# davidedomini/experiments-2025-acsos-marl-for-swarming-behaviors

Measured on AMD Instinct MI355X. Metric: env-steps/sec (agents×envs), GoTo 8 agents×1024 envs @1/2/4/8 GPU, higher is better.
Workload: dtype f32; 1 GPU; GoTo train tick: 8 agents x 1024 envs/GPU, GAT, complete graph, eps 0.05, TD batch 1024 graphs/GPU; envs_per_gpu=1024, agents=8, global_envs=1024, td_batch_per_gpu=1024, graph=complete, conv=gat, parallelism=env-sharded dp1, hipgraph=True, tick=1 launch + reduce

## Files before the change

### experiments-2025-acsos-marl-for-swarming-behaviors_amd/csrc/swarm_actk.h

```cpp
#pragma once
#include "swarm_adam.h"
#include "swarm_env.h"
#include "swarm_dl.h"
#include "swarm_gat3.h"

namespace swarm {

enum { MODE_Q = 0, MODE_TICK = 1, MODE_ROLLOUT = 2, MODE_STEP = 3 };

struct ActArgs {
  int B, N, scenario, graph, k, conv, env_offset, flags;
  uint32_t k0, k1;
  float radius;
  int net;
  const float* params;
  const float* x;
  const uint8_t* dense;
  const int32_t* actions;
  float* state;
  swarm_replay replay;
  const swarm_ctrl* ctrl;
  swarm_act_out out;
  int n_ticks;
  uint32_t tick0;
// ... 246 lines not shown
      if (pending && tid == 0 && A.grad_norm_out) *A.grad_norm_out = gn;
    }
  } else if (MODE != MODE_STEP && NET == SWARM_NET_GAT3) {
    for (int i = threadIdx.x; i < G3_N_PARAMS; i += 64 * kActWPB) Pw[i] = A.params[i];
  } else if (MODE != MODE_STEP) {
    ParamStage<64 * kActWPB> ps;
    ps.load(A.params, threadIdx.x);
    ps.store(Pw, threadIdx.x);
  }
  __syncthreads();
  const float* P = Pw;
  SWARM_STAMP(1);

  const int n_ticks = (MODE == MODE_ROLLOUT) ? A.n_ticks : 1;
  float rew_sum[CT], hits_sum = 0.0f;
#pragma unroll
  for (int ct = 0; ct < CT; ++ct) rew_sum[ct] = 0.0f;

  for (int it = 0; it < n_ticks; ++it) {
#if SWARM_STAMPS == 1
    const long long t_tick0 = clock64();
#endif
    if (MODE != MODE_Q && kHoist && it > 0) pair_forces();
    if (MODE != MODE_Q) {
#pragma unroll
      for (int ct = 0; ct < CT; ++ct) {
        node_x(px[ct], py[ct], vx[ct], vy[ct], 16 * ct + c, p, F.x[ct]);
        if (!valid[ct]) { F.x[ct][0] = 0.0f; F.x[ct][1] = 0.0f; }
      }
    }
    if (MODE != MODE_STEP && NET == SWARM_NET_GAT3) {
      gat3_forward<NS>(P, d, N, graph, A.k, A.radius, A.dense, V, F);
    } else if (MODE != MODE_STEP) {
      if constexpr (kDefer) dl_forward<NS, 8, NS>(P, d, N, graph, A.k, A.radius, conv, A.dense, V, false, F, deferred0);
      else dl_forward<NS, 8>(P, d, N, graph, A.k, A.radius, conv, A.dense, V, false, F);
    }
    if constexpr (kDefer) {
      if constexpr (kDeferForces) pair_contacts0();
      if (explore0) {
#pragma unroll
        for (int ct = 0; ct < CT; ++ct) {
          const int agent = min(16 * ct + c, N - 1);
          const u32x4 wd = philox4x32(tick, genv, STREAM_RAND_ACTION, (uint32_t)(agent >> 2), A.k0, A.k1);
          const int j = agent & 3;
          ract0[ct] = uniform_int(j == 0 ? wd.x : (j == 1 ? wd.y : (j == 2 ? wd.z : wd.w)), kActions);
        }
      }
    }
    if (it == 0) SWARM_STAMP(2);

    if (MODE == MODE_Q) {
#pragma unroll
      for (int ct = 0; ct < CT; ++ct)
        if (valid[ct])
          for (int a = p; a < kActions; a += 4) A.out.q[node[ct] * kActions + a] = sm.Q[16 * ct + c][a];
      return;
    }

    const uint32_t tk = tick + (uint32_t)it;
    bool explore = explore0;
    if (it > 0 && eps > 0.0f) explore = u01(philox4x32(tk, genv, STREAM_COIN, 0u, A.k0, A.k1).x) < eps;
    int action[CT];
#pragma unroll
    for (int ct = 0; ct < CT; ++ct) {
      const int agent = min(16 * ct + c, N - 1);
      action[ct] = (MODE == MODE_STEP) ? (valid[ct] ? A.actions[node[ct]] : 0) : argmax9(F.q[ct]);
      if (explore) {
        if (kHoist && it == 0) {
// ... 192 lines not shown
```

### experiments-2025-acsos-marl-for-swarming-behaviors_amd/csrc/swarm_bwd.h

```cpp
#pragma once
#include "swarm_dl.h"

namespace swarm {

constexpr int kTdRows = 32;

template <int NS>
struct TdLds {
  static constexpr int GPB = kTdRows / NS;
  float H[kTdRows][kRow];
  float T[kTdRows][kRow];
  float R[kTdRows][kRow];
  float dZ[kTdRows][kRow];
  float dO[kTdRows][kRow];
  float dH[kTdRows][kRow];
  float X[kTdRows][9];
  union {
    struct {
      float cm[kTdRows][NS + 1];
      float dp[kTdRows][NS + 1];
    };
    WSmall<NS> tgsm[GPB];
  };
  float yq[kTdRows], gq[kTdRows], das[kTdRows], dad[kTdRows], d2[kTdRows];
// ... 30 lines not shown
  for (int t2 = 0; t2 < 2; ++t2)
#pragma unroll
    for (int r = 0; r < 4; ++r) dO[t2][r] = live ? acc[t2][r] * (1.0f - th[t2][r] * th[t2][r]) : 0.0f;
}

template <int NS>
__device__ __forceinline__ void bwd_attention(const float (*H)[kRow], const DFwd<NS>& F, const float* ssrc,
                                              const float (&dO)[DGeom<NS>::CT][2][4], const bool (&live)[DGeom<NS>::CT],
                                              int c, int p, float (&dp)[DGeom<NS>::CT][DGeom<NS>::CT][4],
                                              float (&da_d)[DGeom<NS>::CT]) {
  constexpr int CT = DGeom<NS>::CT;
  static_assert(NS % 16 == 0, "every MFMA column of a wave is one of its node slots");
  float ah[CT][2][4];
#pragma unroll
  for (int ut = 0; ut < CT; ++ut)
#pragma unroll
    for (int t = 0; t < 2; ++t) {
      const float4 hv = *reinterpret_cast<const float4*>(&H[16 * ut + c][16 * t + 4 * p]);
      ah[ut][t][0] = hv.x; ah[ut][t][1] = hv.y; ah[ut][t][2] = hv.z; ah[ut][t][3] = hv.w;
    }
#pragma unroll
  for (int ct = 0; ct < CT; ++ct) {
    float gv[CT][4], cu[CT][4];
    float part = 0.0f;
#pragma unroll
    for (int ut = 0; ut < CT; ++ut) {
      f32x4 acc = {0.f, 0.f, 0.f, 0.f};
#pragma unroll
      for (int t = 0; t < 2; ++t)
#pragma unroll
        for (int r = 0; r < 4; ++r) acc = mfma16(ah[ut][t][r], dO[ct][t][r], acc);
#pragma unroll
      for (int r = 0; r < 4; ++r) {
        float cc[4];
#pragma unroll
        for (int q = 0; q < 4; ++q) cc[q] = F.cf[ct][16 * ut + 4 * q + r];
        cu[ut][r] = pick4(cc, 0, p);
        gv[ut][r] = acc[r];
        part = part + cu[ut][r] * gv[ut][r];
      }
    }
    const float Gs = row4_sum(part);
    float dsum = 0.0f;
#pragma unroll
    for (int ut = 0; ut < CT; ++ut)
#pragma unroll
      for (int r = 0; r < 4; ++r) {
        float dpu = 0.0f;
        if (cu[ut][r] != 0.0f && live[ct]) {
          const float de = cu[ut][r] * (gv[ut][r] - Gs);
          const float pre = ssrc[16 * ut + 4 * p + r] + F.sdst[ct];
          dpu = pre > 0.0f ? de : de * kLeakySlope;
        }
        dsum = dsum + dpu;
        dp[ct][ut][r] = dpu;
      }
    da_d[ct] = row4_sum(dsum);
  }
}

template <int NS, int GS>
__device__ __forceinline__ void bwd_dh(TdLds<NS>& TB, const float* P, int row0, int N, int conv,
                                       const bool (&nv)[DGeom<NS>::CT], const float (&da_d)[DGeom<NS>::CT], int c, int p) {
  constexpr int CT = DGeom<NS>::CT;
  const float4 s0 = *reinterpret_cast<const float4*>(P + L_ATT_SRC + 4 * p);
  const float4 s1 = *reinterpret_cast<const float4*>(P + L_ATT_SRC + 16 + 4 * p);
  const float4 d0 = *reinterpret_cast<const float4*>(P + L_ATT_DST + 4 * p);
  const float4 d1 = *reinterpret_cast<const float4*>(P + L_ATT_DST + 16 + 4 * p);
  const float as[2][4] = {{s0.x, s0.y, s0.z, s0.w}, {s1.x, s1.y, s1.z, s1.w}};
  const float ad[2][4] = {{d0.x, d0.y, d0.z, d0.w}, {d1.x, d1.y, d1.z, d1.w}};
  float ao[2][NS / 4];
#pragma unroll
  for (int t = 0; t < 2; ++t)
#pragma unroll
    for (int ks = 0; ks < NS / 4; ++ks) ao[t][ks] = TB.dO[row0 + 4 * ks + p][16 * t + c];
#pragma unroll
  for (int ct = 0; ct < CT; ++ct) {
    const int u = 16 * ct + c;
    float da_s = 0.0f;
    if (conv == SWARM_CONV_GAT) {
      const int base = (GS < NS) ? (u / GS) * GS : 0;
      float dpj[GS];
#pragma unroll
      for (int j = 0; j < GS; ++j) dpj[j] = TB.dp[row0 + base + j][u];
#pragma unroll
      for (int j = 0; j < GS; ++j) asm volatile("" : "+v"(dpj[j]));
// ... 61 lines not shown
```

### experiments-2025-acsos-marl-for-swarming-behaviors_amd/csrc/swarm_common.h

```cpp
#pragma once
#include <hip/hip_runtime.h>
#include <stdint.h>

#include "../../include/swarm_hip.h"

namespace swarm {

constexpr int kHidden = 32;
constexpr int kFeat = 7;
constexpr int kActions = 9;

constexpr float kGoalX = -0.8f, kGoalY = 0.8f;
constexpr float kObstX = -0.1f, kObstY = 0.1f;
constexpr float kRadius = 0.05f;
constexpr float kCollisionForce = 100.0f;
constexpr float kContactMargin = 0.001f;
constexpr float kMinDist = 1e-6f;
constexpr float kDt = 0.1f;
constexpr float kDragKeep = 0.75f;
constexpr float kLeakySlope = 0.2f;
constexpr float kFlockShaping = 10.0f;
constexpr float kFlockDesired = 0.15f;
constexpr float kFlockContact = 0.005f;
constexpr float kFlockGoalBonus = 50.0f;
// ... 195 lines not shown
    __builtin_amdgcn_sched_barrier(0);                                                        \
    if (g_swarm_stamps && (threadIdx.x & 63) == 0)                                            \
      g_swarm_stamps[((size_t)blockIdx.x * 16 + (threadIdx.x >> 6)) * 32 + (k)] = _t;         \
  } while (0)
#define SWARM_RTSTAMP(k) SWARM_STAMP_AT(k, "s_memrealtime")
#endif
#if SWARM_STAMPS == 1
#define SWARM_STAMP(k) SWARM_STAMP_AT(k, "s_memtime")
#else
#define SWARM_STAMP(k) \
  do {              \
  } while (0)
#endif
#if !SWARM_STAMPS
#define SWARM_RTSTAMP(k) \
  do {                \
  } while (0)
#endif

enum { SPEC_RUNTIME = 0, SPEC_COMPLETE_GAT = 1, SPEC_COMPLETE_GCN = 2, SPEC_KNN_GAT = 3, SPEC_RADIUS_GAT = 4 };
__host__ __device__ inline int spec_of(int graph, int conv) {
  if (graph == SWARM_GRAPH_COMPLETE) return conv == SWARM_CONV_GAT ? SPEC_COMPLETE_GAT : SPEC_COMPLETE_GCN;
  if (graph == SWARM_GRAPH_KNN && conv == SWARM_CONV_GAT) return SPEC_KNN_GAT;
  if (graph == SWARM_GRAPH_RADIUS && conv == SWARM_CONV_GAT) return SPEC_RADIUS_GAT;
  return SPEC_RUNTIME;
}
template <int SPEC>
__device__ inline int spec_graph(int runtime) {
  return SPEC == SPEC_RUNTIME       ? runtime
         : SPEC == SPEC_KNN_GAT     ? (int)SWARM_GRAPH_KNN
         : SPEC == SPEC_RADIUS_GAT  ? (int)SWARM_GRAPH_RADIUS
                                    : (int)SWARM_GRAPH_COMPLETE;
}
template <int SPEC>
__device__ inline int spec_conv(int runtime) {
  return SPEC == SPEC_RUNTIME ? runtime : (SPEC == SPEC_COMPLETE_GCN ? (int)SWARM_CONV_GCN : (int)SWARM_CONV_GAT);
}

}
```

### experiments-2025-acsos-marl-for-swarming-behaviors_amd/csrc/swarm_dl.h

```cpp
#pragma once
#include "swarm_wpg.h"

namespace swarm {

__device__ inline float row4_sum(float x) {
  const int xi = __float_as_int(x);
  const auto a = __builtin_amdgcn_permlane16_swap(xi, xi, false, false);
  const float y = __int_as_float((int)a[0]) + __int_as_float((int)a[1]);
  const int yi = __float_as_int(y);
  const auto b = __builtin_amdgcn_permlane32_swap(yi, yi, false, false);
  return __int_as_float((int)b[0]) + __int_as_float((int)b[1]);
}

template <int M>
__device__ inline float pick4(const float (&v)[M], int k, int p) {
  const float a = v[4 * k], b = v[4 * k + 1], c = v[4 * k + 2], d = v[4 * k + 3];
  return p == 0 ? a : (p == 1 ? b : (p == 2 ? c : d));
}

template <int NS>
struct DGeom {
  static constexpr int CT = (NS + 15) / 16;
  int lane, c, p;
  int gid;
  bool live;
};

template <int NS>
__device__ inline DGeom<NS> make_dgeom(int wave_gid, int count) {
  DGeom<NS> d;
  d.lane = threadIdx.x & 63;
  d.c = d.lane & 15;
  d.p = d.lane >> 4;
  d.live = wave_gid < count;
  d.gid = d.live ? wave_gid : 0;
  return d;
}

template <int NS>
struct DFwd {
  static constexpr int CT = DGeom<NS>::CT;
  float x[CT][2];
  float t[CT][2][4];
  float zr[CT][2][4];
  float cf[CT][NS];
  float sdst[CT];
  float q[CT][kActions];
};

__device__ inline void node_x(float px, float py, float vx, float vy, int agent, int p, float x[2]) {
  x[0] = p == 0 ? px : (p == 1 ? py : (p == 2 ? vx : vy));
  x[1] = p == 0 ? kGoalX : (p == 1 ? kGoalY : (p == 2 ? (float)agent : 0.0f));
}

template <int NS, int GS = NS>
__device__ inline int in_mult(int u, int n, int N, int graph, const WSmall<NS>& sm, const uint8_t* __restrict__ dense,
                              int gid) {
  if constexpr (GS < NS) {
    if (u / GS != n / GS) return 0;
  }
  const int ju = (GS < NS) ? u % GS : u, jn = (GS < NS) ? n % GS : n;
  if (ju >= N || jn >= N) return 0;
  if (graph == SWARM_GRAPH_COMPLETE) return (ju != jn ? 1 : 0) + ((ju == 0 && jn == 0) ? 1 : 0);
  if (graph == SWARM_GRAPH_KNN)
    return (int)((sm.knn[u] >> jn) & 1u) + (int)((sm.knn[n] >> ju) & 1u) + ((ju == 0 && jn == 0) ? 1 : 0);
  if (graph == SWARM_GRAPH_RADIUS)
    return (int)((sm.knn[n] >> ju) & 1u) + ((ju == 0 && jn == 0) ? 1 : 0);
  return (int)dense[((size_t)gid * N + ju) * N + jn];
}

template <int NS, int GS = NS>
__device__ inline void in_mults(int n, int N, int graph, const WSmall<NS>& sm, const uint8_t* __restrict__ dense,
                                int gid, int m[GS]) {
  const int jn = (GS < NS) ? n % GS : n;
  const int base = (GS < NS) ? (n / GS) * GS : 0;
  const bool tv = jn < N;
  if (graph == SWARM_GRAPH_COMPLETE) {
#pragma unroll
    for (int j = 0; j < GS; ++j) m[j] = (tv && j < N) ? (int)(j != jn) + (int)(j == 0 && jn == 0) : 0;
  } else if (graph == SWARM_GRAPH_KNN) {
    const uint32_t kn = sm.knn[min(n, NS - 1)];
#pragma unroll
    for (int j = 0; j < GS; ++j)
      m[j] = (tv && j < N) ? (int)((sm.knn[base + j] >> jn) & 1u) + (int)((kn >> j) & 1u) + (int)(j == 0 && jn == 0) : 0;
  } else if (graph == SWARM_GRAPH_RADIUS) {
    const uint32_t kn = sm.knn[min(n, NS - 1)];
#pragma unroll
    for (int j = 0; j < GS; ++j) m[j] = (tv && j < N) ? (int)((kn >> j) & 1u) + (int)(j == 0 && jn == 0) : 0;
  } else {
#pragma unroll
    for (int j = 0; j < GS; ++j) m[j] = (tv && j < N) ? (int)dense[((size_t)gid * N + j) * N + jn] : 0;
  }
}

template <int NS, int GS = NS>
__device__ inline uint32_t radius_mask_node(int n, int N, float r, const WSmall<NS>& sm) {
  const int base = (GS < NS) ? (n / GS) * GS : 0;
  const int jn = (GS < NS) ? n % GS : n;
  if (jn >= N) return 0u;
  const float xi = sm.px[n], yi = sm.py[n];
  uint32_t m = 0u;
#pragma unroll
  for (int j = 0; j < GS; ++j) {
    const float d = norm2(sm.px[base + j] - xi, sm.py[base + j] - yi);
    m |= (j < N && j != jn && d <= r) ? (1u << j) : 0u;
  }
  return m;
}

template <int NS, int GS = NS>
__device__ inline uint32_t knn_mask_node(int n, int N, int k, const WSmall<NS>& sm, KV* q) {
  float d[GS];
// ... 173 lines not shown
  const unsigned long long tb = __ballot(run);
  if (tb != 0ull) {
#if SWARM_STAMPS == 1
    const long long s0 = clock64();
#endif
    wave_lds_sync();
    knn_tie_rows_wave<NS, GS>(lane, N, k, tb, LPN, sm, dn, q);
    wave_lds_sync();
    if (memo && run) {
      memo->sig_lo[n] = sig_lo;
      memo->sig_hi[n] = sig_hi;
      memo->mask[n] = sm.knn[n];
    }
#if SWARM_STAMPS == 1
    wave_lds_sync();
    const long long s1 = clock64();
    if (g_swarm_stamps && lane == 0) {
      unsigned long long* ws = g_swarm_stamps + ((size_t)blockIdx.x * 16 + (threadIdx.x >> 6)) * 32;
      ws[27] += 1ull;
      ws[28] += (unsigned long long)(s1 - s0);
      if ((unsigned long long)(s1 - s0) > ws[26]) ws[26] = (unsigned long long)(s1 - s0);
    }
#endif
  }
#if SWARM_STAMPS == 1
  if (memo && g_swarm_stamps && lane == 0 && __ballot(hit) != 0ull)
    g_swarm_stamps[((size_t)blockIdx.x * 16 + (threadIdx.x >> 6)) * 32 + 18] += 1ull;
#endif
}

struct DlNoHook {
  __device__ __forceinline__ void operator()() const {}
};
template <int NS, int SB = -1, int GS = NS, class HOOK = DlNoHook>
__device__ inline void dl_forward(const float* __restrict__ P, const DGeom<NS>& d, int N, int graph, int k, float radius, int conv,
                                  const uint8_t* __restrict__ dense, const WView<NS>& V, bool keep_tr, DFwd<NS>& F,
                                  const HOOK& hook = HOOK()) {
#define DF_STAMP(i) do { if (SB >= 0) SWARM_STAMP(SB + (i)); } while (0)
  constexpr int CT = DGeom<NS>::CT;
  WSmall<NS>& sm = *V.sm;
  const int c = d.c, p = d.p;
  float h[CT][2][4];
  {
    float a0[2][2];
#pragma unroll
    for (int t = 0; t < 2; ++t) {
      a0[t][0] = P[L_W + (16 * t + c) * kFeat + p];
      a0[t][1] = P[L_W + (16 * t + c) * kFeat + 4 + p];
      asm volatile("" : "+v"(a0[t][1]));
      a0[t][1] = (4 + p < kFeat) ? a0[t][1] : 0.0f;
    }
#pragma unroll
    for (int ct = 0; ct < CT; ++ct)
#pragma unroll
      for (int t = 0; t < 2; ++t) {
        f32x4 acc = {0.f, 0.f, 0.f, 0.f};
        acc = mfma16(a0[t][0], F.x[ct][0], acc);
        acc = mfma16(a0[t][1], F.x[ct][1], acc);
#pragma unroll
        for (int r = 0; r < 4; ++r) h[ct][t][r] = acc[r];
      }
  }
  float ssrc[CT];
  {
    const float4 s0 = *reinterpret_cast<const float4*>(P + L_ATT_SRC + 4 * p);
    const float4 s1 = *reinterpret_cast<const float4*>(P + L_ATT_SRC + 16 + 4 * p);
    const float4 d0 = *reinterpret_cast<const float4*>(P + L_ATT_DST + 4 * p);
// ... 13 lines not shown
  }
#pragma unroll
  for (int ct = 0; ct < CT; ++ct) {
    const int n = 16 * ct + c;
    if (n < NS) {
      *reinterpret_cast<float4*>(&V.H[n][4 * p]) = make_float4(h[ct][0][0], h[ct][0][1], h[ct][0][2], h[ct][0][3]);
      *reinterpret_cast<float4*>(&V.H[n][16 + 4 * p]) = make_float4(h[ct][1][0], h[ct][1][1], h[ct][1][2], h[ct][1][3]);
      if (p == 0) { sm.ssrc[n] = ssrc[ct]; sm.sdst[n] = F.sdst[ct]; sm.px[n] = F.x[ct][0]; }
      if (p == 1) sm.py[n] = F.x[ct][0];
    }
  }
  wave_lds_sync();
  DF_STAMP(0);
  if (graph == SWARM_GRAPH_KNN) {
    if constexpr (NS <= 16) {
      knn_masks_wave<NS, GS>(d.lane, N, k, sm, &V.T[0][0], reinterpret_cast<KV*>(&V.R[0][0]), V.memo);
    } else {
#pragma unroll
      for (int ct = 0; ct < CT; ++ct) {
        const int n = 16 * ct + c;
        KV* q = reinterpret_cast<KV*>(&V.T[0][0]) + (n < NS ? n : 0) * GS;
        if (n < NS && p == 0) sm.knn[n] = (((GS < NS) ? n % GS : n) < N) ? knn_mask_node<NS, GS>(n, N, k, sm, q) : 0u;
      }
    }
    wave_lds_sync();
  } else if (graph == SWARM_GRAPH_RADIUS) {
#pragma unroll
    for (int ct = 0; ct < CT; ++ct) {
      const int n = 16 * ct + c;
      if (n < NS && p == 0) sm.knn[n] = radius_mask_node<NS, GS>(n, N, radius, sm);
    }
    wave_lds_sync();
  }
  if (conv == SWARM_CONV_GAT) {
#pragma unroll
    for (int ct = 0; ct < CT; ++ct) {
      const int n = 16 * ct + c, base = (GS < NS) ? (n / GS) * GS : 0;
      float e[GS];
      int m[GS];
      in_mults<NS, GS>(n, N, graph, sm, dense, d.gid, m);
      float mx[GS];
#pragma unroll
      for (int j = 0; j < GS; ++j) {
        e[j] = leaky(sm.ssrc[base + j] + F.sdst[ct]);
        mx[j] = m[j] > 0 ? e[j] : -INFINITY;
      }
#pragma unroll
      for (int w = GS / 2; w >= 1; w >>= 1)
#pragma unroll
        for (int j = 0; j < w; ++j) mx[j] = fmaxf(mx[j], mx[j + w]);
      const float emax = mx[0];
      float den = 0.0f;
#pragma unroll
      for (int j = 0; j < GS; ++j) {
        e[j] = m[j] > 0 ? __expf(e[j] - emax) : 0.0f;
        den = den + (float)m[j] * e[j];
      }
      den = den + 1e-16f;
      const float inv = 1.0f / den;
      float cl[GS];
#pragma unroll
      for (int j = 0; j < GS; ++j) cl[j] = (float)m[j] * (e[j] * inv);
#pragma unroll
      for (int u = 0; u < NS; ++u) F.cf[ct][u] = (GS == NS || u / GS == n / GS) ? cl[u % GS] : 0.0f;
    }
  } else {
    float dis[CT];
#pragma unroll
    for (int ct = 0; ct < CT; ++ct) {
      const int n = 16 * ct + c, base = (GS < NS) ? (n / GS) * GS : 0;
      float deg = 0.0f;
#pragma unroll
      for (int j = 0; j < GS; ++j)
        if (j < N) deg = deg + (base + j == n ? 1.0f : (float)in_mult<NS, GS>(base + j, n, N, graph, sm, dense, d.gid));
      const int jn = (GS < NS) ? n % GS : n;
      dis[ct] = (jn < N && deg > 0.0f) ? 1.0f / sqrtf(deg) : 0.0f;
      if (n < NS && p == 0) sm.aux[n] = dis[ct];
    }
    wave_lds_sync();
#pragma unroll
    for (int ct = 0; ct < CT; ++ct) {
      const int n = 16 * ct + c;
#pragma unroll
      for (int u = 0; u < NS; ++u) {
        const bool same = (GS == NS) || (u / GS == n / GS);
        const float w = (u == n) ? 1.0f : (float)in_mult<NS, GS>(u, n, N, graph, sm, dense, d.gid);
        const int ju = (GS < NS) ? u % GS : u, jn = (GS < NS) ? n % GS : n;
        F.cf[ct][u] = (same && ju < N && jn < N) ? (sm.aux[u] * w) * dis[ct] : 0.0f;
      }
    }
  }
  DF_STAMP(1);
  {
    float ah[2][NS / 4];
#pragma unroll
    for (int t = 0; t < 2; ++t)
#pragma unroll
      for (int ks = 0; ks < NS / 4; ++ks) ah[t][ks] = V.H[4 * ks + p][16 * t + c];
    const float4 b0 = *reinterpret_cast<const float4*>(P + L_BIAS + 4 * p);
    const float4 b1 = *reinterpret_cast<const float4*>(P + L_BIAS + 16 + 4 * p);
    const float bias[2][4] = {{b0.x, b0.y, b0.z, b0.w}, {b1.x, b1.y, b1.z, b1.w}};
#pragma unroll
    for (int ct = 0; ct < CT; ++ct) {
      f32x4 o0 = {0.f, 0.f, 0.f, 0.f}, o1 = {0.f, 0.f, 0.f, 0.f};
#pragma unroll
      for (int ks = 0; ks < NS / 4; ++ks) {
        const float b = pick4(F.cf[ct], ks, p);
        o0 = mfma16(ah[0][ks], b, o0);
        o1 = mfma16(ah[1][ks], b, o1);
      }
#pragma unroll
      for (int r = 0; r < 4; ++r) {
        F.t[ct][0][r] = tanh_fast(o0[r] + bias[0][r]);
        F.t[ct][1][r] = tanh_fast(o1[r] + bias[1][r]);
      }
      const int n = 16 * ct + c;
      if (keep_tr && n < NS) {
        *reinterpret_cast<float4*>(&V.T[n][4 * p]) = make_float4(F.t[ct][0][0], F.t[ct][0][1], F.t[ct][0][2], F.t[ct][0][3]);
        *reinterpret_cast<float4*>(&V.T[n][16 + 4 * p]) = make_float4(F.t[ct][1][0], F.t[ct][1][1], F.t[ct][1][2], F.t[ct][1][3]);
      }
    }
  }
  DF_STAMP(2);
  {
    float a1[2][2][4];
#pragma unroll
    for (int t2 = 0; t2 < 2; ++t2)
#pragma unroll
      for (int t = 0; t < 2; ++t) {
        const float4 w = *reinterpret_cast<const float4*>(P + L_W1 + (16 * t2 + c) * kWRow + 16 * t + 4 * p);
        a1[t2][t][0] = w.x; a1[t2][t][1] = w.y; a1[t2][t][2] = w.z; a1[t2][t][3] = w.w;
      }
    const float4 bb0 = *reinterpret_cast<const float4*>(P + L_B1 + 4 * p);
    const float4 bb1 = *reinterpret_cast<const float4*>(P + L_B1 + 16 + 4 * p);
    const float b1v[2][4] = {{bb0.x, bb0.y, bb0.z, bb0.w}, {bb1.x, bb1.y, bb1.z, bb1.w}};
    hook();
#pragma unroll
    for (int ct = 0; ct < CT; ++ct) {
      f32x4 z[2] = {{0.f, 0.f, 0.f, 0.f}, {0.f, 0.f, 0.f, 0.f}};
#pragma unroll
      for (int t = 0; t < 2; ++t)
#pragma unroll
        for (int r = 0; r < 4; ++r)
#pragma unroll
          for (int t2 = 0; t2 < 2; ++t2) z[t2] = mfma16(a1[t2][t][r], F.t[ct][t][r], z[t2]);
#pragma unroll
      for (int t2 = 0; t2 < 2; ++t2) {
// ... 55 lines not shown
```

### experiments-2025-acsos-marl-for-swarming-behaviors_amd/csrc/swarm_qbk.h

```cpp
#pragma once
#include "swarm_bwd.h"

namespace swarm {

struct QbArgs {
  int B, N, graph, k, conv;
  float radius;
  const float* params;
  const float* x;
  const uint8_t* mult;
  const float* dq;
  float* slabs;
  int n_slabs;
};

constexpr int kQbDqRow = 12;

template <int NS>
struct QbSmem {
  TdLds<NS> TB;
  __attribute__((aligned(16))) float Pon[N_LDS_PARAMS];
  __attribute__((aligned(16))) float DQ[kTdRows][kQbDqRow];
};

// ... 14 lines not shown
  const int conv = spec_conv<SPEC>(A.conv);
  const int row0 = wi * NS;
  const WView<NS> V{TB.H + row0, TB.T + row0, TB.R + row0, &TB.on[wi]};
  static_assert(kSlabCols == 16, "slab column blocks of 16");
  float* const slab_base = A.slabs + (size_t)vb * kSlabCols;
  const uint32_t slab_stride = (uint32_t)A.n_slabs * kSlabCols;
  auto sst = [&](int q, float v) { slab_base[(uint32_t)(q >> 4) * slab_stride + (uint32_t)(q & 15)] = v; };

  ParamStage<NT> pon;
  pon.load(A.params, threadIdx.x);
  bool nv[CT];
  DFwd<NS> F;
  float dqv[CT][kActions];
#pragma unroll
  for (int ct = 0; ct < CT; ++ct) {
    const int n = 16 * ct + c;
    const int gi = (GS < NS) ? n / GS : 0;
    const int jl = (GS < NS) ? n % GS : n;
    const int sid = vb * (kTdRows / GS) + wi * GPW + gi;
    nv[ct] = sid < B && jl < N;
    const size_t node = (size_t)min(sid, B - 1) * N + min(jl, N - 1);
    const float x0 = A.x[node * kFeat + p], x1 = A.x[node * kFeat + min(4 + p, kFeat - 1)];
    F.x[ct][0] = nv[ct] ? x0 : 0.0f;
    F.x[ct][1] = (nv[ct] && 4 + p < kFeat) ? x1 : 0.0f;
#pragma unroll
    for (int a = 0; a < kActions; ++a) {
      const float g = A.dq[node * kActions + a];
      dqv[ct][a] = nv[ct] ? g : 0.0f;
    }
  }
  pon.store(L.Pon, threadIdx.x);
  __syncthreads();

  dl_forward<NS, -1, GS>(P, d, N, graph, A.k, A.radius, conv, A.mult, V, true, F);

  float dz[CT][2][4];
#pragma unroll
  for (int ct = 0; ct < CT; ++ct) {
    float dr[2][4] = {{0.f, 0.f, 0.f, 0.f}, {0.f, 0.f, 0.f, 0.f}};
#pragma unroll
    for (int a = 0; a < kActions; ++a)
#pragma unroll
      for (int t = 0; t < 2; ++t) {
        const float4 w = *reinterpret_cast<const float4*>(P + L_W2 + a * kWRow + 16 * t + 4 * p);
        dr[t][0] = dr[t][0] + w.x * dqv[ct][a];
        dr[t][1] = dr[t][1] + w.y * dqv[ct][a];
        dr[t][2] = dr[t][2] + w.z * dqv[ct][a];
        dr[t][3] = dr[t][3] + w.w * dqv[ct][a];
      }
#pragma unroll
    for (int t = 0; t < 2; ++t)
#pragma unroll
      for (int r = 0; r < 4; ++r) dz[ct][t][r] = (nv[ct] && F.zr[ct][t][r] > 0.0f) ? dr[t][r] : 0.0f;
    const int row = row0 + 16 * ct + c;
    row_store(TB.dZ[row], p, dz[ct]);
    TB.X[row][p] = F.x[ct][0];
    TB.X[row][4 + p] = F.x[ct][1];
#pragma unroll
    for (int j = 0; j < NS / 4; ++j) TB.cm[row][4 * j + p] = pick4(F.cf[ct], j, p);
    if (p == 0) {
      TB.X[row][8] = 0.0f;
      *reinterpret_cast<float4*>(&L.DQ[row][0]) = make_float4(dqv[ct][0], dqv[ct][1], dqv[ct][2], dqv[ct][3]);
    } else if (p == 1) {
      *reinterpret_cast<float4*>(&L.DQ[row][4]) = make_float4(dqv[ct][4], dqv[ct][5], dqv[ct][6], dqv[ct][7]);
    } else if (p == 2) {
      *reinterpret_cast<float4*>(&L.DQ[row][8]) = make_float4(dqv[ct][8], 0.0f, 0.0f, 0.0f);
    }
  }

  float dO[CT][2][4];
#pragma unroll
  for (int ct = 0; ct < CT; ++ct) {
    bwd_dO_tile(P, c, p, dz[ct], F.t[ct], nv[ct], dO[ct]);
    row_store(TB.dO[row0 + 16 * ct + c], p, dO[ct]);
  }
  float da_d[CT];
#pragma unroll
  for (int ct = 0; ct < CT; ++ct) da_d[ct] = 0.0f;
  if (conv == SWARM_CONV_GAT) {
    float dp[CT][CT][4];
    bwd_attention<NS>(TB.H + row0, F, V.sm->ssrc, dO, nv, c, p, dp, da_d);
#pragma unroll
    for (int ct = 0; ct < CT; ++ct)
#pragma unroll
      for (int ut = 0; ut < CT; ++ut)
#pragma unroll
        for (int r = 0; r < 4; ++r) TB.dp[row0 + 16 * ct + c][16 * ut + 4 * p + r] = dp[ct][ut][r];
  }
  wave_lds_sync();
  bwd_dh<NS, GS>(TB, P, row0, N, conv, nv, da_d, c, p);
  __syncthreads();

// ... 59 lines not shown
```

### experiments-2025-acsos-marl-for-swarming-behaviors_amd/csrc/swarm_tdk.h

```cpp
#pragma once
#include "swarm_adam.h"
#include "swarm_bwd.h"
#include "swarm_diag.h"

namespace swarm {

struct TdArgs {
  int S, B, N, graph, k, conv, env_offset;
  uint32_t k0, k1;
  float radius;
  const float* params;
  const float* target;
  swarm_replay replay;
  const swarm_ctrl* ctrl;
  const int32_t* sample_in;
  int32_t* sample_out;
  float* slabs;
  float gamma;
  float grad_scale;
  int n_slabs;
};

__device__ inline void slab_st(float* p, float v) { *p = v; }

// ... 232 lines not shown
        okc[ct] = true;
        if (ho[ct]) {
          okc[ct] = !kHoForceDrop && !(kHoDropTarget && !online) && (uint32_t)(g[ct][0] >> 32) == tag &&
                    (uint32_t)(g[ct][1] >> 32) == tag && (uint32_t)(g[ct][2] >> 32) == tag &&
                    (uint32_t)(g[ct][3] >> 32) == tag;
          ok = ok && okc[ct];
          st[ct] = make_float4(__uint_as_float((uint32_t)g[ct][0]), __uint_as_float((uint32_t)g[ct][1]),
                               __uint_as_float((uint32_t)g[ct][2]), __uint_as_float((uint32_t)g[ct][3]));
        }
      }
      if (!__builtin_amdgcn_ballot_w64(!ok)) break;
      if (kHoForceDrop || (kHoDropTarget && !online) || spin >= kHoSpinLimit) {
        drop_overrun<NS, GS>(okc, live_drop, nv, c);
        if (FUSED && !online && p == 0) {
#pragma unroll
          for (int ct = 0; ct < CT; ++ct)
            if (live_drop[ct]) *(volatile int*)&TB.tdrop[row0 + 16 * ct + c] = 1;
        }
        if (lane == 0) atomicAdd(X.ho_err, 1u);
        break;
      }
      __builtin_amdgcn_s_sleep(SWARM_HO_SLEEP);
    }
    SWARM_RTSTAMP(10);
    __builtin_amdgcn_s_setprio(3);
  }
  DFwd<NS> F;
#pragma unroll
  for (int ct = 0; ct < CT; ++ct) {
    node_x(st[ct].x, st[ct].y, st[ct].z, st[ct].w, jl[ct], p, F.x[ct]);
    if (!nv[ct]) { F.x[ct][0] = 0.0f; F.x[ct][1] = 0.0f; }
  }
  if (!online && !waited) __builtin_amdgcn_s_setprio(2);
  dl_forward<NS, 16, GS>(online ? Pon : Ptg, d, N, graph, A.k, A.radius, conv, nullptr, V, online, F);
  if (FUSED && waited && online) {
    for (int spin = 0;; ++spin) {
      bool ok = true, okc[CT];
#pragma unroll
      for (int ct = 0; ct < CT; ++ct) {
        okc[ct] = true;
        if (ho[ct] && !live_drop[ct]) {
          const unsigned long long g = ld_granule(ho_at(ct, 9 * N, 1));
          okc[ct] = !kHoForceDrop && (uint32_t)(g >> 32) == tag;
          ok = ok && okc[ct];
          act[ct] = nv[ct] ? (int)(uint32_t)g : 0;
        }
      }
      if (!__builtin_amdgcn_ballot_w64(!ok)) break;
      if (kHoForceDrop || spin >= kHoSpinLimit) {
        if (lane == 0) atomicAdd(X.ho_err, 1u);
        drop_overrun<NS, GS>(okc, live_drop, nv, c);
        break;
      }
      __builtin_amdgcn_s_sleep(1);
    }
    if (p == 0) {
#pragma unroll
      for (int ct = 0; ct < CT; ++ct) TB.act[row0 + 16 * ct + c] = nv[ct] ? act[ct] : 0;
    }
  }
  float dO1[CT][2][4], dp1[CT][CT][4], dad1[CT];
  if (pre) {
#pragma unroll
    for (int ct = 0; ct < CT; ++ct) {
      const int ac = min(max(act[ct], 0), kActions - 1);
      float dz1[2][4];
#pragma unroll
// ... 58 lines not shown
      if (FUSED) TB.tdrop[row0 + 16 * ct + c] = live_drop[ct] ? 1 : 0;
    }
  }
  if (!online && !waited) __builtin_amdgcn_s_setprio(0);
  if (online && lane == 0) TB.prew[wi] = pre ? 1 : 0;
  SWARM_STAMP(3);
  __syncthreads();
  SWARM_STAMP(4);

  const float* P = Pon;
  float dz[CT][2][4];
  if (online) {
#pragma unroll
    for (int ct = 0; ct < CT; ++ct) {
      const int row = row0 + 16 * ct + c;
      if (FUSED && TB.tdrop[row]) nv[ct] = false;
      float qa = F.q[ct][0];
#pragma unroll
      for (int a = 1; a < kActions; ++a) qa = (act[ct] == a) ? F.q[ct][a] : qa;
      const float delta = nv[ct] ? (qa - (rew[ct] + TB.yq[row])) : 0.0f;
      const float gq = delta * A.grad_scale;
#pragma unroll
      for (int t = 0; t < 2; ++t) {
        const float4 w = *reinterpret_cast<const float4*>(P + L_W2 + act[ct] * kWRow + 16 * t + 4 * p);
        float wv[4] = {w.x, w.y, w.z, w.w};
        asm volatile("" : "+v"(wv[0]), "+v"(wv[1]), "+v"(wv[2]), "+v"(wv[3]));
#pragma unroll
        for (int r = 0; r < 4; ++r) dz[ct][t][r] = F.zr[ct][t][r] > 0.0f ? wv[r] * gq : 0.0f;
      }
      row_store(TB.dZ[row], p, dz[ct]);
      TB.X[row][p] = F.x[ct][0];
      TB.X[row][4 + p] = F.x[ct][1];
#pragma unroll
      for (int j = 0; j < NS / 4; ++j) TB.cm[row][4 * j + p] = pick4(F.cf[ct], j, p);
      if (p == 0) { TB.X[row][8] = 0.0f; TB.gq[row] = gq; TB.d2[row] = delta * delta; }
      if (pre) {
        float o[2][4];
#pragma unroll
        for (int t = 0; t < 2; ++t)
#pragma unroll
          for (int r = 0; r < 4; ++r) o[t][r] = nv[ct] ? dO1[ct][t][r] * gq : 0.0f;
        row_store(TB.dO[row], p, o);
        if (conv == SWARM_CONV_GAT) {
#pragma unroll
          for (int ut = 0; ut < CT; ++ut)
#pragma unroll
            for (int r = 0; r < 4; ++r) TB.dp[row][16 * ut + 4 * p + r] = nv[ct] ? dp1[ct][ut][r] * gq : 0.0f;
        }
        dad1[ct] = nv[ct] ? dad1[ct] * gq : 0.0f;
      }
    }
  }
  __syncthreads();
  SWARM_STAMP(5);
  int np_pre = 0;
#pragma unroll
  for (int w2 = 0; w2 < GPB; ++w2) np_pre += TB.prew[w2];
  auto b2_tiles = [&](int tj) {
    float a1[2][8], b1[8], a2[8], b2v[8];
    int an[8];
#pragma unroll
    for (int s = 0; s < 8; ++s) {
      const int n = 4 * s + p;
      a1[0][s] = TB.dZ[n][c];
      a1[1][s] = TB.dZ[n][16 + c];
      b1[s] = TB.T[n][16 * tj + c];
      b2v[s] = TB.R[n][16 * tj + c];
// ... 101 lines not shown
```

Baseline: 625.7 million agent-steps/s.

## Compute only lane-picked GAT coefficients and specialise complete-graph softmax

Replaces the full per-node coefficient table (cf[CT][NS]) with only the entries each lane actually consumes: column picks for the aggregation MFMA and row picks for the backward attention. The picks are selected with a two-level select, and compile-time proofs check that they match the original table. A UNIT template path for complete-graph specs drops the integer multiplicity arrays and multiplies, deriving edges from a constexpr predicate. The aggregation MFMAs are also split from the tanh epilogue. The aim is to cut register pressure and per-lane ALU work in the forward pass used by the act, TD and Q-backward kernels, at the cost of more template complexity.

Result: faster. 638.1 million agent-steps/s, median of 6 (+2.0%).

```diff
diff --git a/experiments-2025-acsos-marl-for-swarming-behaviors_amd/csrc/swarm_actk.h b/experiments-2025-acsos-marl-for-swarming-behaviors_amd/csrc/swarm_actk.h
--- a/experiments-2025-acsos-marl-for-swarming-behaviors_amd/csrc/swarm_actk.h
+++ b/experiments-2025-acsos-marl-for-swarming-behaviors_amd/csrc/swarm_actk.h
@@ -302,8 +302,8 @@
     if (MODE != MODE_STEP && NET == SWARM_NET_GAT3) {
       gat3_forward<NS>(P, d, N, graph, A.k, A.radius, A.dense, V, F);
     } else if (MODE != MODE_STEP) {
-      if constexpr (kDefer) dl_forward<NS, 8, NS>(P, d, N, graph, A.k, A.radius, conv, A.dense, V, false, F, deferred0);
-      else dl_forward<NS, 8>(P, d, N, graph, A.k, A.radius, conv, A.dense, V, false, F);
+      if constexpr (kDefer) dl_forward<NS, 8, NS, spec_complete_graph(SPEC)>(P, d, N, graph, A.k, A.radius, conv, A.dense, V, false, F, deferred0);
+      else dl_forward<NS, 8, NS, spec_complete_graph(SPEC)>(P, d, N, graph, A.k, A.radius, conv, A.dense, V, false, F);
     }
     if constexpr (kDefer) {
       if constexpr (kDeferForces) pair_contacts0();
diff --git a/experiments-2025-acsos-marl-for-swarming-behaviors_amd/csrc/swarm_bwd.h b/experiments-2025-acsos-marl-for-swarming-behaviors_amd/csrc/swarm_bwd.h
--- a/experiments-2025-acsos-marl-for-swarming-behaviors_amd/csrc/swarm_bwd.h
+++ b/experiments-2025-acsos-marl-for-swarming-behaviors_amd/csrc/swarm_bwd.h
@@ -86,10 +86,7 @@
         for (int r = 0; r < 4; ++r) acc = mfma16(ah[ut][t][r], dO[ct][t][r], acc);
 #pragma unroll
       for (int r = 0; r < 4; ++r) {
-        float cc[4];
-#pragma unroll
-        for (int q = 0; q < 4; ++q) cc[q] = F.cf[ct][16 * ut + 4 * q + r];
-        cu[ut][r] = pick4(cc, 0, p);
+        cu[ut][r] = F.cr[ct][ut][r];
         gv[ut][r] = acc[r];
         part = part + cu[ut][r] * gv[ut][r];
       }
@@ -100,12 +97,10 @@
     for (int ut = 0; ut < CT; ++ut)
 #pragma unroll
       for (int r = 0; r < 4; ++r) {
-        float dpu = 0.0f;
-        if (cu[ut][r] != 0.0f && live[ct]) {
-          const float de = cu[ut][r] * (gv[ut][r] - Gs);
-          const float pre = ssrc[16 * ut + 4 * p + r] + F.sdst[ct];
-          dpu = pre > 0.0f ? de : de * kLeakySlope;
-        }
+        const float de = cu[ut][r] * (gv[ut][r] - Gs);
+        const float pre = ssrc[16 * ut + 4 * p + r] + F.sdst[ct];
+        const float dpe = pre > 0.0f ? de : de * kLeakySlope;
+        const float dpu = (cu[ut][r] != 0.0f && live[ct]) ? dpe : 0.0f;
         dsum = dsum + dpu;
         dp[ct][ut][r] = dpu;
       }
diff --git a/experiments-2025-acsos-marl-for-swarming-behaviors_amd/csrc/swarm_common.h b/experiments-2025-acsos-marl-for-swarming-behaviors_amd/csrc/swarm_common.h
--- a/experiments-2025-acsos-marl-for-swarming-behaviors_amd/csrc/swarm_common.h
+++ b/experiments-2025-acsos-marl-for-swarming-behaviors_amd/csrc/swarm_common.h
@@ -251,6 +251,7 @@
          : SPEC == SPEC_RADIUS_GAT  ? (int)SWARM_GRAPH_RADIUS
                                     : (int)SWARM_GRAPH_COMPLETE;
 }
+constexpr bool spec_complete_graph(int spec) { return spec == SPEC_COMPLETE_GAT || spec == SPEC_COMPLETE_GCN; }
 template <int SPEC>
 __device__ inline int spec_conv(int runtime) {
   return SPEC == SPEC_RUNTIME ? runtime : (SPEC == SPEC_COMPLETE_GCN ? (int)SWARM_CONV_GCN : (int)SWARM_CONV_GAT);
diff --git a/experiments-2025-acsos-marl-for-swarming-behaviors_amd/csrc/swarm_dl.h b/experiments-2025-acsos-marl-for-swarming-behaviors_amd/csrc/swarm_dl.h
--- a/experiments-2025-acsos-marl-for-swarming-behaviors_amd/csrc/swarm_dl.h
+++ b/experiments-2025-acsos-marl-for-swarming-behaviors_amd/csrc/swarm_dl.h
@@ -1,4 +1,6 @@
 #pragma once
+#include <type_traits>
+
 #include "swarm_wpg.h"
 
 namespace swarm {
@@ -12,11 +14,54 @@
   return __int_as_float((int)b[0]) + __int_as_float((int)b[1]);
 }
 
-template <int M>
-__device__ inline float pick4(const float (&v)[M], int k, int p) {
-  const float a = v[4 * k], b = v[4 * k + 1], c = v[4 * k + 2], d = v[4 * k + 3];
-  return p == 0 ? a : (p == 1 ? b : (p == 2 ? c : d));
-}
+template <class T>
+__device__ __forceinline__ T sel4(bool b0, bool b1, T x0, T x1, T x2, T x3) {
+  const T lo = b0 ? x1 : x0, hi = b0 ? x3 : x2;
+  return b1 ? hi : lo;
+}
+
+template <int NS, int GS>
+struct CoefPick {
+  static constexpr int CT = (NS + 15) / 16;
+  static_assert(GS % 4 == 0 && NS % GS == 0, "a pick's four candidates lie in one graph, 1 or 4 apart");
+  static constexpr int col_j(int ks, int q) { return (4 * ks) % GS + q; }
+  static constexpr int col_g(int ks) { return (4 * ks) / GS; }
+  static constexpr int row_j(int ut, int q, int r) { return (16 * ut + 4 * q) % GS + r; }
+  static constexpr int row_g(int ut, int q) { return (16 * ut + 4 * q) / GS; }
+  static constexpr bool same(int u, int n) { return u / GS == n / GS; }
+  static constexpr bool proved() {
+    for (int ct = 0; ct < CT; ++ct)
+      for (int c = 0; c < 16; ++c)
+        for (int p = 0; p < 4; ++p) {
+          const int n = 16 * ct + c;
+          for (int ks = 0; ks < NS / 4; ++ks) {
+            const int u = 4 * ks + p, j = col_j(ks, p);
+            if (j < 0 || j >= GS) return false;
+            if ((col_g(ks) == n / GS) != same(u, n)) return false;
+            if (same(u, n) && j != u % GS) return false;
+          }
+          if (NS % 16 != 0) continue;
+          for (int ut = 0; ut < CT; ++ut)
+            for (int r = 0; r < 4; ++r) {
+              const int u = 16 * ut + 4 * p + r, j = row_j(ut, p, r);
+              if (u >= NS || j < 0 || j >= GS) return false;
+              if ((row_g(ut, p) == n / GS) != same(u, n)) return false;
+              if (same(u, n) && j != u % GS) return false;
+            }
+        }
+    return true;
+  }
+};
+
+constexpr int complete_mult(int j, int jn) { return (int)(j != jn) + (int)(j == 0 && jn == 0); }
+constexpr bool complete_edge(int j, int jn) { return j == 0 || j != jn; }
+constexpr bool complete_mult_is_edge(int gs) {
+  for (int j = 0; j < gs; ++j)
+    for (int jn = 0; jn < gs; ++jn)
+      if (complete_mult(j, jn) != (complete_edge(j, jn) ? 1 : 0)) return false;
+  return true;
+}
+static_assert(complete_mult_is_edge(32), "complete graph: multiplicity == in-edge predicate, 0 or 1");
 
 template <int NS>
 struct DGeom {
@@ -43,7 +88,8 @@
   float x[CT][2];
   float t[CT][2][4];
   float zr[CT][2][4];
-  float cf[CT][NS];
+  float cc[CT][NS / 4];
+  float cr[CT][CT][4];
   float sdst[CT];
   float q[CT][kActions];
 };
@@ -77,7 +123,7 @@
   const bool tv = jn < N;
   if (graph == SWARM_GRAPH_COMPLETE) {
 #pragma unroll
-    for (int j = 0; j < GS; ++j) m[j] = (tv && j < N) ? (int)(j != jn) + (int)(j == 0 && jn == 0) : 0;
+    for (int j = 0; j < GS; ++j) m[j] = (tv && j < N) ? complete_mult(j, jn) : 0;
   } else if (graph == SWARM_GRAPH_KNN) {
     const uint32_t kn = sm.knn[min(n, NS - 1)];
 #pragma unroll
@@ -317,7 +363,7 @@
 struct DlNoHook {
   __device__ __forceinline__ void operator()() const {}
 };
-template <int NS, int SB = -1, int GS = NS, class HOOK = DlNoHook>
+template <int NS, int SB = -1, int GS = NS, bool UNIT = false, class HOOK = DlNoHook>
 __device__ inline void dl_forward(const float* __restrict__ P, const DGeom<NS>& d, int N, int graph, int k, float radius, int conv,
                                   const uint8_t* __restrict__ dense, const WView<NS>& V, bool keep_tr, DFwd<NS>& F,
                                   const HOOK& hook = HOOK()) {
@@ -397,47 +443,82 @@
     }
     wave_lds_sync();
   }
+  using CP = CoefPick<NS, GS>;
+  static_assert(CP::proved(), "the lane's coefficient picks name the full table's entries");
+  const bool pb0 = (p & 1) != 0, pb1 = (p & 2) != 0;
   if (conv == SWARM_CONV_GAT) {
-#pragma unroll
-    for (int ct = 0; ct < CT; ++ct) {
-      const int n = 16 * ct + c, base = (GS < NS) ? (n / GS) * GS : 0;
-      float e[GS];
-      int m[GS];
-      in_mults<NS, GS>(n, N, graph, sm, dense, d.gid, m);
-      float mx[GS];
-#pragma unroll
-      for (int j = 0; j < GS; ++j) {
-        e[j] = leaky(sm.ssrc[base + j] + F.sdst[ct]);
-        mx[j] = m[j] > 0 ? e[j] : -INFINITY;
-      }
-#pragma unroll
-      for (int w = GS / 2; w >= 1; w >>= 1)
-#pragma unroll
-        for (int j = 0; j < w; ++j) mx[j] = fmaxf(mx[j], mx[j + w]);
-      const float emax = mx[0];
-      float den = 0.0f;
-#pragma unroll
-      for (int j = 0; j < GS; ++j) {
-        e[j] = m[j] > 0 ? __expf(e[j] - emax) : 0.0f;
-        den = den + (float)m[j] * e[j];
-      }
-      den = den + 1e-16f;
-      const float inv = 1.0f / den;
-      float cl[GS];
-#pragma unroll
-      for (int j = 0; j < GS; ++j) cl[j] = (float)m[j] * (e[j] * inv);
-#pragma unroll
-      for (int u = 0; u < NS; ++u) F.cf[ct][u] = (GS == NS || u / GS == n / GS) ? cl[u % GS] : 0.0f;
+    {
+#pragma unroll
+      for (int ct = 0; ct < CT; ++ct) {
+        const int n = 16 * ct + c, base = (GS < NS) ? (n / GS) * GS : 0;
+        const int ng = (GS < NS) ? n / GS : 0;
+        float e[GS];
+        int m[GS];
+        bool in[GS];
+        if constexpr (UNIT) {
+          const int jn = (GS < NS) ? n % GS : n;
+#pragma unroll
+          for (int j = 0; j < GS; ++j) { in[j] = jn < N && j < N && complete_edge(j, jn); m[j] = 0; }
+        } else {
+          in_mults<NS, GS>(n, N, graph, sm, dense, d.gid, m);
+#pragma unroll
+          for (int j = 0; j < GS; ++j) in[j] = m[j] > 0;
+        }
+        float mx[GS];
+#pragma unroll
+        for (int j = 0; j < GS; ++j) {
+          e[j] = leaky(sm.ssrc[base + j] + F.sdst[ct]);
+          mx[j] = in[j] ? e[j] : -INFINITY;
+        }
+#pragma unroll
+        for (int w = GS / 2; w >= 1; w >>= 1)
+#pragma unroll
+          for (int j = 0; j < w; ++j) mx[j] = fmaxf(mx[j], mx[j + w]);
+        const float emax = mx[0];
+        float den = 0.0f;
+#pragma unroll
+        for (int j = 0; j < GS; ++j) {
+          e[j] = in[j] ? __expf(e[j] - emax) : 0.0f;
+          den = UNIT ? den + e[j] : den + (float)m[j] * e[j];
+        }
+        den = den + 1e-16f;
+        const float inv = 1.0f / den;
+        auto coef = [&](float ep, int mp, bool same) -> float {
+          const float v = UNIT ? ep * inv : (float)mp * (ep * inv);
+          return same ? v : 0.0f;
+        };
+#pragma unroll
+        for (int ks = 0; ks < NS / 4; ++ks) {
+          const int j0 = CP::col_j(ks, 0), j1 = CP::col_j(ks, 1), j2 = CP::col_j(ks, 2), j3 = CP::col_j(ks, 3);
+          float v = coef(sel4(pb0, pb1, e[j0], e[j1], e[j2], e[j3]), sel4(pb0, pb1, m[j0], m[j1], m[j2], m[j3]),
+                         GS == NS || CP::col_g(ks) == ng);
+          asm volatile("" : "+v"(v));
+          F.cc[ct][ks] = v;
+        }
+        if constexpr (NS % 16 == 0) {
+#pragma unroll
+          for (int ut = 0; ut < CT; ++ut)
+#pragma unroll
+            for (int r = 0; r < 4; ++r) {
+              const int j0 = CP::row_j(ut, 0, r), j1 = CP::row_j(ut, 1, r), j2 = CP::row_j(ut, 2, r), j3 = CP::row_j(ut, 3, r);
+              F.cr[ct][ut][r] = coef(sel4(pb0, pb1, e[j0], e[j1], e[j2], e[j3]), sel4(pb0, pb1, m[j0], m[j1], m[j2], m[j3]),
+                                     GS == NS || CP::row_g(ut, p) == ng);
+            }
+        }
+      }
     }
   } else {
     float dis[CT];
+    float wl[CT][GS];
 #pragma unroll
     for (int ct = 0; ct < CT; ++ct) {
       const int n = 16 * ct + c, base = (GS < NS) ? (n / GS) * GS : 0;
       float deg = 0.0f;
 #pragma unroll
-      for (int j = 0; j < GS; ++j)
-        if (j < N) deg = deg + (base + j == n ? 1.0f : (float)in_mult<NS, GS>(base + j, n, N, graph, sm, dense, d.gid));
+      for (int j = 0; j < GS; ++j) {
+        wl[ct][j] = base + j == n ? 1.0f : (float)in_mult<NS, GS>(base + j, n, N, graph, sm, dense, d.gid);
+        if (j < N) deg = deg + wl[ct][j];
+      }
       const int jn = (GS < NS) ? n % GS : n;
       dis[ct] = (jn < N && deg > 0.0f) ? 1.0f / sqrtf(deg) : 0.0f;
       if (n < NS && p == 0) sm.aux[n] = dis[ct];
@@ -445,13 +526,14 @@
     wave_lds_sync();
 #pragma unroll
     for (int ct = 0; ct < CT; ++ct) {
-      const int n = 16 * ct + c;
-#pragma unroll
-      for (int u = 0; u < NS; ++u) {
-        const bool same = (GS == NS) || (u / GS == n / GS);
-        const float w = (u == n) ? 1.0f : (float)in_mult<NS, GS>(u, n, N, graph, sm, dense, d.gid);
-        const int ju = (GS < NS) ? u % GS : u, jn = (GS < NS) ? n % GS : n;
-        F.cf[ct][u] = (same && ju < N && jn < N) ? (sm.aux[u] * w) * dis[ct] : 0.0f;
+      const int n = 16 * ct + c, jn = (GS < NS) ? n % GS : n, ng = (GS < NS) ? n / GS : 0;
+#pragma unroll
+      for (int ks = 0; ks < NS / 4; ++ks) {
+        const int j0 = CP::col_j(ks, 0), j1 = CP::col_j(ks, 1), j2 = CP::col_j(ks, 2), j3 = CP::col_j(ks, 3);
+        const float w = sel4(pb0, pb1, wl[ct][j0], wl[ct][j1], wl[ct][j2], wl[ct][j3]);
+        const int u = 4 * ks + p, ju = j0 + p;
+        const bool same = GS == NS || CP::col_g(ks) == ng;
+        F.cc[ct][ks] = (same && ju < N && jn < N) ? (sm.aux[u] * w) * dis[ct] : 0.0f;
       }
     }
   }
@@ -465,19 +547,24 @@
     const float4 b0 = *reinterpret_cast<const float4*>(P + L_BIAS + 4 * p);
     const float4 b1 = *reinterpret_cast<const float4*>(P + L_BIAS + 16 + 4 * p);
     const float bias[2][4] = {{b0.x, b0.y, b0.z, b0.w}, {b1.x, b1.y, b1.z, b1.w}};
-#pragma unroll
-    for (int ct = 0; ct < CT; ++ct) {
-      f32x4 o0 = {0.f, 0.f, 0.f, 0.f}, o1 = {0.f, 0.f, 0.f, 0.f};
+    f32x4 o0[CT], o1[CT];
+#pragma unroll
+    for (int ct = 0; ct < CT; ++ct) {
+      o0[ct] = f32x4{0.f, 0.f, 0.f, 0.f};
+      o1[ct] = f32x4{0.f, 0.f, 0.f, 0.f};
 #pragma unroll
       for (int ks = 0; ks < NS / 4; ++ks) {
-        const float b = pick4(F.cf[ct], ks, p);
-        o0 = mfma16(ah[0][ks], b, o0);
-        o1 = mfma16(ah[1][ks], b, o1);
-      }
+        const float b = F.cc[ct][ks];
+        o0[ct] = mfma16(ah[0][ks], b, o0[ct]);
+        o1[ct] = mfma16(ah[1][ks], b, o1[ct]);
+      }
+    }
+#pragma unroll
+    for (int ct = 0; ct < CT; ++ct) {
 #pragma unroll
       for (int r = 0; r < 4; ++r) {
-        F.t[ct][0][r] = tanh_fast(o0[r] + bias[0][r]);
-        F.t[ct][1][r] = tanh_fast(o1[r] + bias[1][r]);
+        F.t[ct][0][r] = tanh_fast(o0[ct][r] + bias[0][r]);
+        F.t[ct][1][r] = tanh_fast(o1[ct][r] + bias[1][r]);
       }
       const int n = 16 * ct + c;
       if (keep_tr && n < NS) {
diff --git a/experiments-2025-acsos-marl-for-swarming-behaviors_amd/csrc/swarm_qbk.h b/experiments-2025-acsos-marl-for-swarming-behaviors_amd/csrc/swarm_qbk.h
--- a/experiments-2025-acsos-marl-for-swarming-behaviors_amd/csrc/swarm_qbk.h
+++ b/experiments-2025-acsos-marl-for-swarming-behaviors_amd/csrc/swarm_qbk.h
@@ -70,7 +70,7 @@
   pon.store(L.Pon, threadIdx.x);
   __syncthreads();
 
-  dl_forward<NS, -1, GS>(P, d, N, graph, A.k, A.radius, conv, A.mult, V, true, F);
+  dl_forward<NS, -1, GS, spec_complete_graph(SPEC)>(P, d, N, graph, A.k, A.radius, conv, A.mult, V, true, F);
 
   float dz[CT][2][4];
 #pragma unroll
@@ -95,7 +95,7 @@
     TB.X[row][p] = F.x[ct][0];
     TB.X[row][4 + p] = F.x[ct][1];
 #pragma unroll
-    for (int j = 0; j < NS / 4; ++j) TB.cm[row][4 * j + p] = pick4(F.cf[ct], j, p);
+    for (int j = 0; j < NS / 4; ++j) TB.cm[row][4 * j + p] = F.cc[ct][j];
     if (p == 0) {
       TB.X[row][8] = 0.0f;
       *reinterpret_cast<float4*>(&L.DQ[row][0]) = make_float4(dqv[ct][0], dqv[ct][1], dqv[ct][2], dqv[ct][3]);
diff --git a/experiments-2025-acsos-marl-for-swarming-behaviors_amd/csrc/swarm_tdk.h b/experiments-2025-acsos-marl-for-swarming-behaviors_amd/csrc/swarm_tdk.h
--- a/experiments-2025-acsos-marl-for-swarming-behaviors_amd/csrc/swarm_tdk.h
+++ b/experiments-2025-acsos-marl-for-swarming-behaviors_amd/csrc/swarm_tdk.h
@@ -288,7 +288,7 @@
     if (!nv[ct]) { F.x[ct][0] = 0.0f; F.x[ct][1] = 0.0f; }
   }
   if (!online && !waited) __builtin_amdgcn_s_setprio(2);
-  dl_forward<NS, 16, GS>(online ? Pon : Ptg, d, N, graph, A.k, A.radius, conv, nullptr, V, online, F);
+  dl_forward<NS, 16, GS, spec_complete_graph(SPEC)>(online ? Pon : Ptg, d, N, graph, A.k, A.radius, conv, nullptr, V, online, F);
   if (FUSED && waited && online) {
     for (int spin = 0;; ++spin) {
       bool ok = true, okc[CT];
@@ -413,7 +413,7 @@
       TB.X[row][p] = F.x[ct][0];
       TB.X[row][4 + p] = F.x[ct][1];
 #pragma unroll
-      for (int j = 0; j < NS / 4; ++j) TB.cm[row][4 * j + p] = pick4(F.cf[ct], j, p);
+      for (int j = 0; j < NS / 4; ++j) TB.cm[row][4 * j + p] = F.cc[ct][j];
       if (p == 0) { TB.X[row][8] = 0.0f; TB.gq[row] = gq; TB.d2[row] = delta * delta; }
       if (pre) {
         float o[2][4];
```
